# ramanathanlab/distllm

Measured on NVIDIA H100. Metric: embedded chunks/sec @512-tok, higher is better.
Workload: dtype bf16

## Files before the change

distllm_b200/csrc/b2e_api.cu:

```cuda
#include "../../include/b2e.h"
#include "../../include/b2e_debug.h"

#include <cuda.h>
#include <cuda_runtime.h>

#include <cstdarg>
#include <cstdio>
#include <cstdlib>
#include <cstring>
#include <string>
#include <utility>
#include <vector>

#include "attention.cuh"
#include "binsearch.cuh"
#include "common.cuh"
#include "gemm.cuh"
#include "mistral_ops.cuh"
#include "pack.cuh"
#include "rowops.cuh"
#include "topk.cuh"
#include "topk_tc.cuh"

using namespace b2e;
// ... 63 lines not shown
  return B2E_OK;
}

int make_tmap_codes(CUtensorMap* tm, const void* base, uint64_t rows, uint64_t cols) {
  EncodeTiledFn fn = get_encode_fn();
  if (!fn) return fail(B2E_ERR_CUDA, "cuTensorMapEncodeTiled entry point unavailable");
  cuuint64_t dims[2] = {cols, rows};
  cuuint64_t strides[1] = {cols};
  cuuint32_t box[2] = {GEMM_BK / 2, GEMM_BN};
  cuuint32_t estr[2] = {1, 1};
  CUresult r = fn(tm, CU_TENSOR_MAP_DATA_TYPE_UINT8, 2, const_cast<void*>(base), dims, strides, box, estr,
                  CU_TENSOR_MAP_INTERLEAVE_NONE, CU_TENSOR_MAP_SWIZZLE_NONE, CU_TENSOR_MAP_L2_PROMOTION_L2_256B,
                  CU_TENSOR_MAP_FLOAT_OOB_FILL_NONE);
  if (r != CUDA_SUCCESS)
    return fail(B2E_ERR_CUDA, "cuTensorMapEncodeTiled codes(rows=%llu, cols=%llu) -> %d", (unsigned long long)rows,
                (unsigned long long)cols, (int)r);
  return B2E_OK;
}

int make_tmap_f32(CUtensorMap* tm, const void* base, uint64_t rows, uint64_t cols, uint32_t box_rows) {
  EncodeTiledFn fn = get_encode_fn();
  if (!fn) return fail(B2E_ERR_CUDA, "cuTensorMapEncodeTiled entry point unavailable");
  cuuint64_t dims[2] = {cols, rows};
  cuuint64_t strides[1] = {cols * 4};
  cuuint32_t box[2] = {32, box_rows};
  cuuint32_t estr[2] = {1, 1};
  CUresult r = fn(tm, CU_TENSOR_MAP_DATA_TYPE_FLOAT32, 2, const_cast<void*>(base), dims, strides, box, estr,
                  CU_TENSOR_MAP_INTERLEAVE_NONE, CU_TENSOR_MAP_SWIZZLE_128B, CU_TENSOR_MAP_L2_PROMOTION_L2_256B,
                  CU_TENSOR_MAP_FLOAT_OOB_FILL_NONE);
  if (r != CUDA_SUCCESS)
    return fail(B2E_ERR_CUDA, "cuTensorMapEncodeTiled f32(rows=%llu, cols=%llu, box_rows=%u) -> %d",
                (unsigned long long)rows, (unsigned long long)cols, box_rows, (int)r);
  return B2E_OK;
}

struct DeviceInfo {
  int sms = 0;
  int cc_major = 0;
  bool ok = false;
};

int device_info(int device, DeviceInfo* info) {
  int n = 0;
  if (cudaGetDeviceCount(&n) != cudaSuccess || n == 0) {
    cudaGetLastError();
    return fail(B2E_ERR_NO_DEVICE, "no CUDA device visible; libb2e has no CPU fallback");
  }
  if (device < 0 || device >= n) return fail(B2E_ERR_INVALID, "device %d out of range", device);
  cudaDeviceProp p;
  CUDA_TRY(cudaGetDeviceProperties(&p, device));
  if (p.major != 9 || p.minor != 0)
    return fail(B2E_ERR_NO_DEVICE, "device %d is sm_%d%d; libb2e is built for sm_90a only", device,
                p.major, p.minor);
  info->sms = p.multiProcessorCount;
  info->cc_major = p.major;
  info->ok = true;
  return B2E_OK;
}

int current_device_info(DeviceInfo* info) {
  int dev = 0;
  if (cudaGetDevice(&dev) != cudaSuccess) {
    cudaGetLastError();
    return fail(B2E_ERR_NO_DEVICE, "no CUDA device visible; libb2e has no CPU fallback");
  }
  static DeviceInfo cache[64];
  if (dev < 64 && cache[dev].ok) {
    *info = cache[dev];
    return B2E_OK;
  }
  int rc = device_info(dev, info);
  if (rc == B2E_OK && dev < 64) cache[dev] = *info;
  return rc;
}

template <typename Kern>
int ensure_smem_attr(Kern kern, int bytes) {
  static std::vector<std::pair<const void*, int>> done;
  int dev = 0;
  CUDA_TRY(cudaGetDevice(&dev));
  const void* key = reinterpret_cast<const void*>(kern);
  for (const auto& d : done)
    if (d.first == key && d.second == dev) return B2E_OK;
  CUDA_TRY(cudaFuncSetAttribute(kern, cudaFuncAttributeMaxDynamicSharedMemorySize, bytes));
  done.emplace_back(key, dev);
  return B2E_OK;
}

int check_gemm_shape(int M, int N, int K) {
  if (M <= 0 || N <= 0 || K <= 0) return fail(B2E_ERR_INVALID, "gemm: empty shape %dx%dx%d", M, N, K);
  if (N % 128 != 0) return fail(B2E_ERR_INVALID, "gemm: N=%d must be a multiple of 128", N);
  if (K % 64 != 0) return fail(B2E_ERR_INVALID, "gemm: K=%d must be a multiple of 64", K);
  return B2E_OK;
}

bool g_gemm_profiling = false;

int g_gemm_bn = -1;
inline int gemm_bn_override() {
  if (g_gemm_bn < 0) {
    const char* e = getenv("B2E_GEMM_BN");
    const int v = e ? atoi(e) : 0;
    g_gemm_bn = (v == 128 || v == 192) ? v : 0;
  }
  return g_gemm_bn;
}

int gemm_bn(int N, int epi, bool nf4) {
  const bool wide_ok = !nf4 && epi != B2E_EPI_SWIGLU && epi != B2E_EPI_GEGLU && N % 192 == 0;
  if (!wide_ok) return 128;
  const int forced = gemm_bn_override();
  return forced ? forced : 192;
}

struct GemmW {
  CUtensorMap tm;
  const float* absmax = nullptr;
  int bn = GEMM_BN;
};

int make_gemm_w(GemmW* w, const void* base, const float* absmax, uint64_t rows, uint64_t cols, int epi) {
  w->absmax = absmax;
  w->bn = gemm_bn((int)rows, epi, absmax != nullptr);
  return absmax ? make_tmap_codes(&w->tm, base, rows, cols / 2) : make_tmap_h16(&w->tm, base, rows, cols, w->bn);
}

template <int EPI>
int launch_gemm_epi(const CUtensorMap& ta, const GemmW& wb, void* out, const float* bias,
                    const h16* resid, int M, int N, int K, cudaStream_t st, const int* m_dev) {
  auto kern = gemm_h16_wgmma_kernel<EPI>;
  int smem = GEMM_SMEM_BYTES;
  if (N % wb.bn != 0) return fail(B2E_ERR_INVALID, "gemm: N=%d is not a multiple of its W map's tile width %d", N, wb.bn);
  if (wb.absmax) {
    kern = gemm_h16_wgmma_kernel<EPI, false, true>;
    smem = GemmPlan<true>::SMEM_BYTES;
  } else if (wb.bn == 192) {
    if constexpr (epi_is_glu(EPI)) {
      return fail(B2E_ERR_INVALID, "gemm: the gated epilogues run 128-wide tiles only");
    } else {
      kern = gemm_h16_wgmma_kernel<EPI, false, false, 192>;
      smem = GemmPlan<false, 192>::SMEM_BYTES;
      if constexpr (EPI == EPI_BIAS)
        if (g_gemm_profiling) kern = gemm_h16_wgmma_kernel<EPI, true, false, 192>;
    }
  } else if constexpr (EPI == EPI_BIAS) {
    if (g_gemm_profiling) kern = gemm_h16_wgmma_kernel<EPI, true>;
  }
  int rc = ensure_smem_attr(kern, smem);
  if (rc) return rc;
  DeviceInfo dev;
  if ((rc = current_device_info(&dev))) return rc;
  const long long tiles = (long long)(N / wb.bn) * ((M + GEMM_BM - 1) / GEMM_BM);
  if (tiles > 0x7fffffffLL) return fail(B2E_ERR_INVALID, "gemm: %lld output tiles exceed one grid", tiles);
  CUtensorMap tm_out;
  if ((rc = make_tmap_h16(&tm_out, out, M, epi_is_glu(EPI) ? N / 2 : N, GEMM_BM))) return rc;
  const unsigned grid = (unsigned)(tiles < dev.sms ? tiles : dev.sms);
  kern<<<grid, GEMM_THREADS, smem, st>>>(ta, wb.tm, tm_out, static_cast<h16*>(out), bias, resid, M, N, K, m_dev,
                                         wb.absmax);
  CUDA_TRY(cudaGetLastError());
  return B2E_OK;
}

int launch_gemm(const CUtensorMap& ta, const GemmW& tb, void* out, const float* bias,
                const void* resid, int M, int N, int K, int epi, cudaStream_t st, const int* m_dev = nullptr) {
  const h16* r = static_cast<const h16*>(resid);
  switch (epi) {
    case B2E_EPI_BIAS: return launch_gemm_epi<EPI_BIAS>(ta, tb, out, bias, r, M, N, K, st, m_dev);
    case B2E_EPI_BIAS_GELU: return launch_gemm_epi<EPI_BIAS_GELU>(ta, tb, out, bias, r, M, N, K, st, m_dev);
    case B2E_EPI_BIAS_RESID: return launch_gemm_epi<EPI_BIAS_RESID>(ta, tb, out, bias, r, M, N, K, st, m_dev);
    case B2E_EPI_SWIGLU: return launch_gemm_epi<EPI_SWIGLU>(ta, tb, out, bias, r, M, N, K, st, m_dev);
    case B2E_EPI_GEGLU: return launch_gemm_epi<EPI_GEGLU>(ta, tb, out, bias, r, M, N, K, st, m_dev);
  }
  return fail(B2E_ERR_INVALID, "unknown epilogue %d", epi);
}

template <typename T>
struct DevBuf {
  T* p = nullptr;
  size_t cap = 0;
  operator T*() const { return p; }
  int grow(size_t n, uint64_t& gen, bool zero = false) {
    if (n <= cap) return B2E_OK;
    ++gen;
    release();
    CUDA_TRY(cudaMalloc(&p, n * sizeof(T)));
    if (zero) CUDA_TRY(cudaMemset(p, 0, n * sizeof(T)));
    cap = n;
    return B2E_OK;
  }
  void release() {
    cudaFree(p);
    p = nullptr;
    cap = 0;
  }
};

struct DeviceScratch {
  int device = -1;
  uint64_t gen = 0;
};

template <typename Scratch>
int follow_device(Scratch& s) {
  int dev = 0;
  CUDA_TRY(cudaGetDevice(&dev));
  if (dev != s.device) {
    s.release();
    s.device = dev;
    ++s.gen;
  }
  return B2E_OK;
}

struct AttnScratch : DeviceScratch {
  DevBuf<float> bias;
  DevBuf<int> kv_chunks;
  DevBuf<int> plain_chunks;
  int ensure(int B, int S_pad) {
    int rc;
    if ((rc = follow_device(*this)) || (rc = bias.grow((size_t)B * S_pad, gen)) || (rc = kv_chunks.grow(B, gen)) ||
        (rc = plain_chunks.grow(B, gen)))
      return rc;
    return B2E_OK;
  }
  void release() {
    bias.release();
    kv_chunks.release();
    plain_chunks.release();
  }
};

inline int attn_s_pad(int S) { return (S + AT_KC - 1) / AT_KC * AT_KC; }

int attention_prepare(AttnScratch& sc, const int64_t* mask, int B, int S, cudaStream_t st) {
  int rc;
  const int S_pad = attn_s_pad(S);
  if ((rc = sc.ensure(B, S_pad))) return rc;
  attn_prep_kernel<<<(B + 7) / 8, 256, 0, st>>>(mask, sc.bias, sc.kv_chunks, sc.plain_chunks, B, S, S_pad);
  CUDA_TRY(cudaGetLastError());
  return B2E_OK;
}

struct SeqLayout {
  const int* cu = nullptr;
  const int* len = nullptr;
  const int* t_real = nullptr;
  const int* tok_src = nullptr;
};

struct PackBuffers : DeviceScratch {
  DevBuf<int> len_raw, ok, len;
  DevBuf<int> cu;
  DevBuf<int> t_real;
  DevBuf<int> src;
  int ensure(int B, size_t tokens) {
    int rc;
    if ((rc = follow_device(*this)) || (rc = len_raw.grow(B, gen)) || (rc = ok.grow(B, gen)) ||
        (rc = len.grow(B, gen)) || (rc = cu.grow((size_t)B + 1, gen)) || (rc = t_real.grow(2, gen)) ||
        (rc = src.grow(tokens, gen)))
      return rc;
    return B2E_OK;
  }
  void release() {
    len_raw.release(); ok.release(); len.release(); cu.release(); t_real.release(); src.release();
  }
};

template <int D, int MODE, int V>
int launch_attention_kernel(const CUtensorMap& tm, const AttnScratch& sc, void* ctx, int B, int S, int heads,
                            int kv_heads, int window, cudaStream_t st, const SeqLayout& lay) {
  using Cfg = AtCfg<D, V>;
  auto kern = attention_kernel<D, MODE, V>;
  int rc = ensure_smem_attr(kern, Cfg::SMEM_BYTES);
  if (rc) return rc;
  CUtensorMap tm_ctx = {};
  if ((V & 128) && (rc = make_tmap_h16(&tm_ctx, ctx, (uint64_t)B * S, (uint64_t)heads * D, 64, Cfg::COLS))) return rc;
  const float scale_log2e = 1.4426950408889634f / sqrtf(static_cast<float>(D));
  const long long ctas = (long long)heads * B * ((S + Cfg::QT - 1) / Cfg::QT);
  if (ctas > 0x7fffffffLL)
    return fail(B2E_ERR_INVALID, "attention: %lld CTAs (heads=%d B=%d S=%d) exceed one grid", ctas, heads, B, S);
  kern<<<(unsigned)ctas, Cfg::THREADS, Cfg::SMEM_BYTES, st>>>(tm, tm_ctx, sc.bias, sc.kv_chunks, sc.plain_chunks, B, S,
                                                    attn_s_pad(S), heads, kv_heads, window, scale_log2e, lay.cu,
                                                    lay.len, static_cast<h16*>(ctx));
  CUDA_TRY(cudaGetLastError());
  return B2E_OK;
}

constexpr int AT_DEFAULT_VARIANT = 193;
int g_att3_variant = -1;
inline int att3_variant() {
  if (g_att3_variant < 0) {
    const char* e = getenv("B2E_ATT3");
    g_att3_variant = e ? atoi(e) : AT_DEFAULT_VARIANT;
  }
  return g_att3_variant;
}

int launch_attention(const CUtensorMap& tkv, const AttnScratch& sc, void* ctx, int B, int S, int heads,
                     cudaStream_t st, int window = 0, const SeqLayout& lay = SeqLayout()) {
  const int v = att3_variant();
#define B2E_ATT(MODE, V) launch_attention_kernel<64, MODE, V>(tkv, sc, ctx, B, S, heads, heads, window, st, lay)
  if (window > 0) {
    switch (v & 192) {
      case 0: return B2E_ATT(1, 0);
      case 64: return B2E_ATT(1, 64);
      case 128: return B2E_ATT(1, 128);
      case 192: return B2E_ATT(1, 192);
    }
    return fail(B2E_ERR_INVALID, "windowed attention: variant %d has no instantiation (bits 6-7 of the variant pick "
                "0, 64, 128 or 192)", v);
  }
// ... 127 lines not shown
  NORM_ADD_RMS,
};

using TrunkFn = int (*)(B2EEncoder* e, const int64_t* ids, const int64_t* mask, const int64_t* types, int B, int S,
                        cudaStream_t st, const SeqLayout& lay);

struct Family {
  int lead, stride;
  int wqkv, wo, w1, w2;
  bool w1_gated;
  int w1_epi;
  FinalNorm norm;
  int norm_g, norm_b;
  TrunkFn trunk;
};
const Family* family(int arch);
}

struct B2EEncoder {
  B2EModelDesc desc;
  const Family* fam = nullptr;
  int full_layers = 0;
  std::vector<const void*> w;
  int device = 0;
  int sms = 0;
  DevBuf<h16> hidden, qkv, ctx, tmp, ffn;
  DevBuf<float> xres, tok_scale;
  PoolScratch pool;
  AttnScratch attn;
  PackBuffers pack;
  std::vector<GemmW> tm_wqkv, tm_wo, tm_w1, tm_w2;
  DevBuf<int64_t> stage_in;
  DevBuf<float> stage_out;
  cudaStream_t own_stream = nullptr;
  float *rope_cos = nullptr, *rope_sin = nullptr;
  float *rope_cos2 = nullptr, *rope_sin2 = nullptr;

  const void* slot(int l, int k) const { return w[fam->lead + fam->stride * l + k]; }
  const float* final_norm(int k) const {
    const int s = k ? fam->norm_b : fam->norm_g;
    if (s < 0) return nullptr;
    return (const float*)(fam->norm == NORM_POST_LN ? slot(desc.num_layers - 1, s) : w[s]);
  }
  struct StepGraph {
    int B, S, pool_kind, l2, has_types, slot;
    cudaGraphExec_t exec;
  };
  std::vector<StepGraph> graphs;
  uint64_t ws_gen = 0;
  uint64_t graphs_stamp = 0;
  uint64_t buffer_stamp() const { return ws_gen + pool.gen + attn.gen + pack.gen; }
  void drop_graphs() {
    for (auto& g : graphs) cudaGraphExecDestroy(g.exec);
    graphs.clear();
  }

  int qkv_cols() const {
    return is_decoder(desc.arch) ? (desc.heads + 2 * desc.kv_heads) * desc.head_dim : 3 * desc.hidden;
  }
  int ctx_cols() const { return is_decoder(desc.arch) ? desc.heads * desc.head_dim : desc.hidden; }
  bool has_xres() const { return desc.arch != B2E_ARCH_BERT; }
};

namespace {

size_t tokens_bytes(const B2EModelDesc& d, size_t tokens) {
  if (is_decoder(d.arch))
    return tokens * (size_t)(2 * d.hidden + (2 * d.heads + 2 * d.kv_heads) * d.head_dim + d.intermediate) * 2;
  return tokens * (size_t)(6 * d.hidden + d.intermediate) * 2;
}

int ensure_workspace(B2EEncoder* e, int B, int S) {
  const size_t tokens = (size_t)B * S, H = e->desc.hidden, I = e->desc.intermediate;
  uint64_t& gen = e->ws_gen;
  int rc;
  if ((rc = e->hidden.grow(tokens * H, gen, true)) || (rc = e->tmp.grow(tokens * H, gen, true)) ||
      (rc = e->qkv.grow(tokens * e->qkv_cols(), gen, true)) || (rc = e->ctx.grow(tokens * e->ctx_cols(), gen, true)) ||
      (rc = e->ffn.grow(tokens * I, gen, true)))
    return rc;
  if (e->has_xres() && (rc = e->xres.grow(tokens * H, gen, true))) return rc;
  if (e->desc.arch == B2E_ARCH_ESM2 && (rc = e->tok_scale.grow(B, gen))) return rc;
  if ((rc = e->pack.ensure(B, tokens))) return rc;
  return e->pool.ensure(B, S, (size_t)B * pool_nsplit(S) * e->desc.hidden);
}

int g_packing = -1;
inline bool packing_enabled() {
  if (g_packing < 0) {
    const char* e = getenv("B2E_PACKED");
    g_packing = (e && e[0] == '0') ? 0 : 1;
  }
  return g_packing == 1;
}

int pack_prepare(PackBuffers& pk, const int64_t* mask, int B, int S, bool enable, cudaStream_t st, SeqLayout* lay) {
  pack_lengths_kernel<<<(B + 7) / 8, 256, 0, st>>>(mask, pk.len_raw, pk.ok, B, S);
  pack_scan_kernel<<<1, 256, 0, st>>>(pk.len_raw, pk.ok, pk.len, pk.cu, pk.t_real, B, S, enable ? 1 : 0);
  pack_fill_kernel<<<dim3((S + 255) / 256, B), 256, 0, st>>>(pk.len, pk.cu, pk.src, B, S);
  CUDA_TRY(cudaGetLastError());
  lay->cu = pk.cu;
  lay->len = pk.len;
  lay->t_real = pk.t_real;
  lay->tok_src = pk.src;
  return B2E_OK;
}

int validate_batch(const B2EEncoder* e, int B, int S) {
  if (!e) return fail(B2E_ERR_INVALID, "null encoder handle");
  if (B <= 0 || S <= 0) return fail(B2E_ERR_INVALID, "empty batch B=%d S=%d", B, S);
  int cur = -1;
  if (cudaGetDevice(&cur) == cudaSuccess && cur != e->device)
    return fail(B2E_ERR_INVALID, "encoder lives on device %d but device %d is current", e->device, cur);
  if (S > e->desc.max_pos)
    return fail(B2E_ERR_INVALID, "S=%d exceeds max_position_embeddings=%d", S, e->desc.max_pos);
  return B2E_OK;
}

struct TrunkMaps {
  CUtensorMap hidden, ctx, ffn, qkv;
};

int trunk_prologue(B2EEncoder* e, const int64_t* mask, int B, int S, cudaStream_t st, TrunkMaps* tm) {
  const B2EModelDesc& d = e->desc;
  const int M = B * S;
  int rc;
  if ((rc = attention_prepare(e->attn, mask, B, S, st))) return rc;
  if ((rc = make_tmap_h16(&tm->hidden, e->hidden, M, d.hidden, 128))) return rc;
  if ((rc = make_tmap_h16(&tm->ctx, e->ctx, M, e->ctx_cols(), 128))) return rc;
  if ((rc = make_tmap_h16(&tm->ffn, e->ffn, M, d.intermediate, 128))) return rc;
  if (is_decoder(d.arch)) return B2E_OK;
  return make_tmap_h16(&tm->qkv, e->qkv, M, e->qkv_cols(), AT_KC, d.head_dim);
}

int run_bert_trunk(B2EEncoder* e, const int64_t* ids, const int64_t* mask, const int64_t* types,
                   int B, int S, cudaStream_t st, const SeqLayout& lay) {
  const B2EModelDesc& d = e->desc;
  const int M = B * S, H = d.hidden, I = d.intermediate;
  int rc;
  DISPATCH_H(H, (embed_layernorm_kernel<HW><<<row_blocks(M), ROW_THREADS, 0, st>>>(
                     ids, types, (const float*)e->w[0], (const float*)e->w[1], (const float*)e->w[2],
                     (const float*)e->w[3], (const float*)e->w[4], e->hidden, M, S, d.eps, lay.t_real,
                     lay.tok_src)));
  CUDA_TRY(cudaGetLastError());

  TrunkMaps tm;
  if ((rc = trunk_prologue(e, mask, B, S, st, &tm))) return rc;

  for (int l = 0; l < d.num_layers; ++l) {
    if ((rc = launch_gemm(tm.hidden, e->tm_wqkv[l], e->qkv, (const float*)e->slot(l, 1), nullptr, M,
                          3 * H, H, B2E_EPI_BIAS, st, lay.t_real)))
      return rc;
    if ((rc = launch_attention_bidir(tm.qkv, e->attn, e->ctx, B, S, d.heads, d.head_dim, st, lay)))
      return rc;
    if ((rc = launch_gemm(tm.ctx, e->tm_wo[l], e->tmp, (const float*)e->slot(l, 3), nullptr, M, H, H,
                          B2E_EPI_BIAS, st, lay.t_real)))
      return rc;
    DISPATCH_H(H, (layernorm_kernel<HW, h16><<<row_blocks(M), ROW_THREADS, 0, st>>>(
                       e->tmp, e->hidden, (const float*)e->slot(l, 4), (const float*)e->slot(l, 5),
                       e->hidden, M, d.eps, lay.t_real)));
    if ((rc = launch_gemm(tm.hidden, e->tm_w1[l], e->ffn, (const float*)e->slot(l, 7), nullptr, M, I,
                          H, B2E_EPI_BIAS_GELU, st, lay.t_real)))
      return rc;
    if ((rc = launch_gemm(tm.ffn, e->tm_w2[l], e->tmp, (const float*)e->slot(l, 9), nullptr, M, H, I,
                          B2E_EPI_BIAS, st, lay.t_real)))
      return rc;
    if (l + 1 < d.num_layers) {
      DISPATCH_H(H, (layernorm_kernel<HW, h16><<<row_blocks(M), ROW_THREADS, 0, st>>>(
                         e->tmp, e->hidden, (const float*)e->slot(l, 10), (const float*)e->slot(l, 11),
                         e->hidden, M, d.eps, lay.t_real)));
    }
  }
  CUDA_TRY(cudaGetLastError());
  return B2E_OK;
}

int run_esm_trunk(B2EEncoder* e, const int64_t* ids, const int64_t* mask, const int64_t*, int B, int S,
                  cudaStream_t st, const SeqLayout& lay) {
  const B2EModelDesc& d = e->desc;
  const int M = B * S, H = d.hidden, I = d.intermediate, L = d.num_layers;
  const int mask_token = d.reserved - 1;
  int rc;
  esm_token_scale_kernel<<<(B + 7) / 8, 256, 0, st>>>(ids, mask, e->tok_scale, B, S, mask_token);
  DISPATCH_H(H, (esm_embed_kernel<HW><<<row_blocks(M), ROW_THREADS, 0, st>>>(
                     ids, mask, (const float*)e->w[0], e->tok_scale, e->xres, M, S, mask_token, lay.t_real,
                     lay.tok_src)));
  CUDA_TRY(cudaGetLastError());
  TrunkMaps tm;
  if ((rc = trunk_prologue(e, mask, B, S, st, &tm))) return rc;

  DISPATCH_H(H, (add_layernorm_kernel<HW, h16><<<row_blocks(M), ROW_THREADS, 0, st>>>(
                     e->xres, nullptr, (const float*)e->slot(0, 0), (const float*)e->slot(0, 1), e->hidden,
                     M, d.eps, lay.t_real)));
  const long long rope_work = (long long)M * d.heads * 2;
  for (int l = 0; l < L; ++l) {
    if ((rc = launch_gemm(tm.hidden, e->tm_wqkv[l], e->qkv, (const float*)e->slot(l, 3), nullptr, M,
                          3 * H, H, B2E_EPI_BIAS, st, lay.t_real)))
      return rc;
    if (d.head_dim == 32) {
      rope_halves_kernel<16><<<(unsigned)((rope_work * 2 + 255) / 256), 256, 0, st>>>(
          e->qkv, e->rope_cos, e->rope_sin, M, S, 2 * d.heads, 3 * H, lay.t_real, lay.tok_src);
    } else {
      rope_halves_kernel<32><<<(unsigned)((rope_work * 4 + 255) / 256), 256, 0, st>>>(
          e->qkv, e->rope_cos, e->rope_sin, M, S, 2 * d.heads, 3 * H, lay.t_real, lay.tok_src);
    }
    if ((rc = launch_attention_bidir(tm.qkv, e->attn, e->ctx, B, S, d.heads, d.head_dim, st, lay)))
      return rc;
    if ((rc = launch_gemm(tm.ctx, e->tm_wo[l], e->tmp, (const float*)e->slot(l, 5), nullptr, M, H, H,
                          B2E_EPI_BIAS, st, lay.t_real)))
      return rc;
    DISPATCH_H(H, (add_layernorm_kernel<HW, h16><<<row_blocks(M), ROW_THREADS, 0, st>>>(
                       e->xres, e->tmp, (const float*)e->slot(l, 6), (const float*)e->slot(l, 7), e->hidden,
                       M, d.eps, lay.t_real)));
    if ((rc = launch_gemm(tm.hidden, e->tm_w1[l], e->ffn, (const float*)e->slot(l, 9), nullptr, M, I, H,
                          B2E_EPI_BIAS_GELU, st, lay.t_real)))
      return rc;
    if ((rc = launch_gemm(tm.ffn, e->tm_w2[l], e->tmp, (const float*)e->slot(l, 11), nullptr, M, H, I,
                          B2E_EPI_BIAS, st, lay.t_real)))
      return rc;
    if (l + 1 < L) {
      DISPATCH_H(H, (add_layernorm_kernel<HW, h16><<<row_blocks(M), ROW_THREADS, 0, st>>>(
                         e->xres, e->tmp, (const float*)e->slot(l + 1, 0), (const float*)e->slot(l + 1, 1),
                         e->hidden, M, d.eps, lay.t_real)));
    }
  }
  CUDA_TRY(cudaGetLastError());
  return B2E_OK;
}

int run_mistral_trunk(B2EEncoder* e, const int64_t* ids, const int64_t* mask, const int64_t*, int B, int S,
                      cudaStream_t st, const SeqLayout& lay) {
  const B2EModelDesc& d = e->desc;
  const int M = B * S, H = d.hidden, I = d.intermediate, L = d.num_layers;
  const int QC = e->qkv_cols(), CC = e->ctx_cols();
  int rc;
  DISPATCH_H(H, (mistral_embed_kernel<HW><<<row_blocks(M), ROW_THREADS, 0, st>>>(
                     ids, (const float*)e->w[0], e->xres, M, lay.t_real, lay.tok_src)));
  CUDA_TRY(cudaGetLastError());
  TrunkMaps tm;
  if ((rc = trunk_prologue(e, mask, B, S, st, &tm))) return rc;

  DISPATCH_H(H, (add_rmsnorm_kernel<HW, h16><<<row_blocks(M), ROW_THREADS, 0, st>>>(
                     e->xres, nullptr, (const float*)e->slot(0, 0), e->hidden, M, d.eps, lay.t_real)));
  const int n_rot = d.heads + d.kv_heads;
  const long long rope_work = (long long)M * n_rot;
  for (int l = 0; l < L; ++l) {
    if ((rc = launch_gemm(tm.hidden, e->tm_wqkv[l], e->qkv, nullptr, nullptr, M, QC, H, B2E_EPI_BIAS, st, lay.t_real)))
      return rc;
    if (d.arch == B2E_ARCH_QWEN3) {
      qk_rmsnorm_rope_kernel<<<(unsigned)((rope_work * 8 + 255) / 256), 256, 0, st>>>(
          e->qkv, (const float*)e->slot(l, 6), (const float*)e->slot(l, 7), e->rope_cos, e->rope_sin, M, S, d.heads,
          d.kv_heads, QC, d.eps, lay.t_real, lay.tok_src);
    } else {
      rope_halves_kernel<64><<<(unsigned)((rope_work * 8 + 255) / 256), 256, 0, st>>>(
          e->qkv, e->rope_cos, e->rope_sin, M, S, n_rot, QC, lay.t_real, lay.tok_src);
    }
    if ((rc = launch_attention_causal_d128(e->qkv, e->attn, e->ctx, B, S, d.heads, d.kv_heads,
                                           d.sliding_window, st, lay)))
      return rc;
    if ((rc = launch_gemm(tm.ctx, e->tm_wo[l], e->tmp, nullptr, nullptr, M, H, CC, B2E_EPI_BIAS, st, lay.t_real)))
      return rc;
    DISPATCH_H(H, (add_rmsnorm_kernel<HW, h16><<<row_blocks(M), ROW_THREADS, 0, st>>>(
                       e->xres, e->tmp, (const float*)e->slot(l, 3), e->hidden, M, d.eps, lay.t_real)));
    if ((rc = launch_gemm(tm.hidden, e->tm_w1[l], e->ffn, nullptr, nullptr, M, 2 * I, H,
                          B2E_EPI_SWIGLU, st, lay.t_real)))
      return rc;
    if ((rc = launch_gemm(tm.ffn, e->tm_w2[l], e->tmp, nullptr, nullptr, M, H, I, B2E_EPI_BIAS, st, lay.t_real)))
      return rc;
    if (l + 1 < L) {
      DISPATCH_H(H, (add_rmsnorm_kernel<HW, h16><<<row_blocks(M), ROW_THREADS, 0, st>>>(
                         e->xres, e->tmp, (const float*)e->slot(l + 1, 0), e->hidden, M, d.eps, lay.t_real)));
    }
  }
  CUDA_TRY(cudaGetLastError());
  return B2E_OK;
}

int run_modernbert_trunk(B2EEncoder* e, const int64_t* ids, const int64_t* mask, const int64_t*, int B, int S,
                         cudaStream_t st, const SeqLayout& lay) {
  const B2EModelDesc& d = e->desc;
  const int M = B * S, H = d.hidden, I = d.intermediate, L = d.num_layers;
  int rc;
  DISPATCH_H(H, (modernbert_embed_kernel<HW><<<row_blocks(M), ROW_THREADS, 0, st>>>(
                     ids, (const float*)e->w[0], (const float*)e->w[1], (const float*)e->w[2], e->xres,
                     e->hidden, M, d.eps, lay.t_real, lay.tok_src)));
  CUDA_TRY(cudaGetLastError());
  TrunkMaps tm;
  if ((rc = trunk_prologue(e, mask, B, S, st, &tm))) return rc;
  const long long rope_work = (long long)M * d.heads * 2;
  for (int l = 0; l < L; ++l) {
    const bool global = (l % d.global_every) == 0;
    if (l > 0) {
      DISPATCH_H(H, (add_layernorm_kernel<HW, h16><<<row_blocks(M), ROW_THREADS, 0, st>>>(
                         e->xres, e->tmp, (const float*)e->slot(l, 0), (const float*)e->slot(l, 1), e->hidden, M,
                         d.eps, lay.t_real)));
    }
    if ((rc = launch_gemm(tm.hidden, e->tm_wqkv[l], e->qkv, nullptr, nullptr, M, 3 * H, H, B2E_EPI_BIAS, st, lay.t_real)))
      return rc;
    rope_halves_kernel<32><<<(unsigned)((rope_work * 4 + 255) / 256), 256, 0, st>>>(
        e->qkv, global ? e->rope_cos : e->rope_cos2, global ? e->rope_sin : e->rope_sin2, M, S, 2 * d.heads,
        3 * H, lay.t_real, lay.tok_src);
    if ((rc = launch_attention(tm.qkv, e->attn, e->ctx, B, S, d.heads, st,
                               global ? 0 : d.sliding_window, lay)))
      return rc;
    if ((rc = launch_gemm(tm.ctx, e->tm_wo[l], e->tmp, nullptr, nullptr, M, H, H, B2E_EPI_BIAS, st, lay.t_real)))
      return rc;
    DISPATCH_H(H, (add_layernorm_kernel<HW, h16><<<row_blocks(M), ROW_THREADS, 0, st>>>(
                       e->xres, e->tmp, (const float*)e->slot(l, 4), (const float*)e->slot(l, 5), e->hidden, M,
                       d.eps, lay.t_real)));
    if ((rc = launch_gemm(tm.hidden, e->tm_w1[l], e->ffn, nullptr, nullptr, M, 2 * I, H, B2E_EPI_GEGLU, st, lay.t_real)))
      return rc;
    if ((rc = launch_gemm(tm.ffn, e->tm_w2[l], e->tmp, nullptr, nullptr, M, H, I, B2E_EPI_BIAS, st, lay.t_real)))
      return rc;
  }
  CUDA_TRY(cudaGetLastError());
  return B2E_OK;
}

constexpr Family kFamilies[] = {
    {5, 12, 0, 2, 6, 8, false, B2E_EPI_BIAS_GELU, NORM_POST_LN, 10, 11, run_bert_trunk},
    {3, 12, 2, 4, 8, 10, false, B2E_EPI_BIAS_GELU, NORM_ADD_LN, 1, 2, run_esm_trunk},
    {2, 6, 1, 2, 4, 5, true, B2E_EPI_SWIGLU, NORM_ADD_RMS, 1, -1, run_mistral_trunk},
// ... 943 lines not shown
```

distllm_b200/csrc/gemm.cuh:

```cuda
#pragma once

#include "common.cuh"

namespace b2e {

enum GemmEpi : int { EPI_BIAS = 0, EPI_BIAS_GELU = 1, EPI_BIAS_RESID = 2, EPI_SWIGLU = 3, EPI_GEGLU = 4 };
__host__ __device__ constexpr bool epi_is_glu(int epi) { return epi == EPI_SWIGLU || epi == EPI_GEGLU; }

constexpr int GEMM_BM = 128;
constexpr int GEMM_BN = 128;
constexpr int GEMM_BK = 64;
constexpr int GEMM_STAGES = 5;
constexpr int GEMM_THREADS = 384;
constexpr int GEMM_PRODUCER_REGS = 40, GEMM_CONSUMER_REGS = 232;
constexpr int GEMM_A_BYTES = GEMM_BM * GEMM_BK * 2;
constexpr int GEMM_STAGE_BYTES = GEMM_A_BYTES + GEMM_BN * GEMM_BK * 2;
constexpr int GEMM_OUT_BOX = GEMM_BM * 64 * 2;
constexpr int GEMM_OUT_OFFSET = GEMM_STAGES * GEMM_STAGE_BYTES;
constexpr int GEMM_BAR_OFFSET = GEMM_OUT_OFFSET + 2 * 2 * GEMM_OUT_BOX;
constexpr int GEMM_SMEM_BYTES = GEMM_BAR_OFFSET + 16 * GEMM_STAGES + 1024;
static_assert(GEMM_SMEM_BYTES <= 232448, "shared memory of one SM");
constexpr int GEMM_BAR_TURN = 1, GEMM_BAR_STAGE = 3, GEMM_BAR_NF4 = 5;

constexpr int GEMM_NF4_RAW = 4;
constexpr int GEMM_NF4_CODE_BYTES = GEMM_BN * GEMM_BK / 2;
constexpr int GEMM_NF4_RAW_BYTES = GEMM_NF4_CODE_BYTES + GEMM_BN * 4;

template <bool NF4, int BN = GEMM_BN>
struct GemmPlan {
  static_assert(BN == 128 || BN == 192, "tile widths");
  static_assert(!NF4 || BN == 128, "the NF4 producer writes one W row per thread of its warpgroup");
  static constexpr int STAGE_BYTES = GEMM_A_BYTES + BN * GEMM_BK * 2;
  static constexpr int OUT_BOXES = BN / 64;
  static constexpr int STAGES = NF4 ? 4 : BN == 192 ? 3 : GEMM_STAGES;
  static constexpr int OUT_OFFSET = STAGES * STAGE_BYTES;
  static constexpr int RAW_OFFSET = OUT_OFFSET + 2 * OUT_BOXES * GEMM_OUT_BOX;
  static constexpr int BAR_OFFSET = RAW_OFFSET + (NF4 ? GEMM_NF4_RAW * GEMM_NF4_RAW_BYTES : 0);
  static constexpr int TABLE_OFFSET = BAR_OFFSET + 16 * STAGES + (NF4 ? 8 * GEMM_NF4_RAW : 0);
  static constexpr int SMEM_BYTES = TABLE_OFFSET + (NF4 ? 16 * 4 : 0) + 1024;
  static constexpr int PRODUCER_REGS = NF4 ? 56 : BN == 192 ? 24 : GEMM_PRODUCER_REGS;
  static constexpr int CONSUMER_REGS = NF4 ? 224 : BN == 192 ? 240 : GEMM_CONSUMER_REGS;
  static_assert(128 * PRODUCER_REGS + 256 * CONSUMER_REGS <= GEMM_THREADS * 168, "registers the CTA holds");
  static_assert(SMEM_BYTES <= 232448, "shared memory of one SM");
};
static_assert(GemmPlan<false>::SMEM_BYTES == GEMM_SMEM_BYTES && GemmPlan<false>::BAR_OFFSET == GEMM_BAR_OFFSET &&
              GemmPlan<false>::STAGE_BYTES == GEMM_STAGE_BYTES, "the 16-bit plan");

__constant__ uint32_t kNf4CodeBits[16] = {
    0xbf800000u, 0xbf3239b1u, 0xbf066b30u, 0xbeca32a0u, 0xbe91a24du, 0xbe3d353fu, 0xbdba7871u, 0x00000000u,
    0x3da2faffu, 0x3e24cae3u, 0x3e7c04ddu, 0x3ead033au, 0x3ee1a4b8u, 0x3f1007abu, 0x3f3913b3u, 0x3f800000u,
};

__device__ __forceinline__ float gelu_erf_fast(float x) {
  const float xc = fminf(fmaxf(x, -5.65685f), 5.65685f);
  const float v = xc * xc;
  float q = fmaf(v, -1.35688221e-05f, -1.95764464e-04f);
  q = fmaf(v, q, 3.65498251e-02f);
  q = fmaf(v, q, 7.97818838e-01f);
  float t;
  asm("tanh.approx.f32 %0, %1;" : "=f"(t) : "f"(xc * q));
  const float h = 0.5f * x;
  return fmaf(h, t, h);
}

__device__ __forceinline__ float gelu_erf(float x) {
  const float ax = fabsf(x);
  float t;
  asm("rcp.approx.ftz.f32 %0, %1;" : "=f"(t) : "f"(fmaf(0.3275911f * 0.70710678f, ax, 1.0f)));
  float p = fmaf(t, 1.061405429f, -1.453152027f);
  p = fmaf(t, p, 1.421413741f);
  p = fmaf(t, p, -0.284496736f);
  p = fmaf(t, p, 0.254829592f);
  p *= t;
  const float e = fast_exp2(ax * ax * (-0.5f * 1.4426950408889634f));
  return fmaxf(x, 0.0f) - 0.5f * ax * p * e;
}

__device__ __forceinline__ float silu(float x) {
  float r;
  asm("rcp.approx.ftz.f32 %0, %1;" : "=f"(r) : "f"(1.0f + fast_exp2(-1.4426950408889634f * x)));
  return x * r;
}


__device__ long long* g_gemm_clock = nullptr;

struct GemmTiles {
  int first, stride, count, n_tiles;
};
template <int BN>
__device__ __forceinline__ GemmTiles gemm_tiles(int M, int N) {
  const int n_tiles = N / BN;
  const int tiles = n_tiles * ((M + GEMM_BM - 1) / GEMM_BM);
  const int first = static_cast<int>(blockIdx.x), stride = static_cast<int>(gridDim.x);
  return {first, stride, first < tiles ? (tiles - 1 - first) / stride + 1 : 0, n_tiles};
}

__device__ __forceinline__ float ld_shared_const_f32(uint32_t addr) {
  float v;
  asm("ld.shared.f32 %0, [%1];" : "=f"(v) : "r"(addr));
  return v;
}
__device__ __forceinline__ float ld_shared_f32(uint32_t addr) {
  float v;
  asm volatile("ld.shared.f32 %0, [%1];" : "=f"(v) : "r"(addr) : "memory");
  return v;
}
__device__ __forceinline__ uint4 ld_shared_v4(uint32_t addr) {
  uint4 v;
  asm volatile("ld.shared.v4.u32 {%0, %1, %2, %3}, [%4];" : "=r"(v.x), "=r"(v.y), "=r"(v.z), "=r"(v.w) : "r"(addr)
               : "memory");
  return v;
}
__device__ __forceinline__ void st_shared_v4(uint32_t addr, uint32_t a, uint32_t b, uint32_t c, uint32_t d) {
  asm volatile("st.shared.v4.b32 [%0], {%1, %2, %3, %4};" ::"r"(addr), "r"(a), "r"(b), "r"(c), "r"(d) : "memory");
}

__device__ __forceinline__ void gemm_nf4_producer(const CUtensorMap* tm_a, const CUtensorMap* tm_codes,
                                                  const float* __restrict__ absmax, const GemmTiles& tl, int N,
                                                  int kblocks, uint32_t sb, uint32_t full_bar, uint32_t empty_bar) {
  using P = GemmPlan<true>;
  const int p = static_cast<int>(threadIdx.x) - 256;
  const uint32_t raw0 = sb + P::RAW_OFFSET;
  const uint32_t raw_bar = empty_bar + 8u * P::STAGES;
  const uint32_t table = sb + P::TABLE_OFFSET;
  const int total = tl.count * kblocks;
  int ld = 0, ld_tile = 0, ld_kb = 0;
  auto load_raw = [&]() {
    const int slot = ld % GEMM_NF4_RAW;
    const int tile = tl.first + ld_tile * tl.stride;
    const int n0 = (tile % tl.n_tiles) * GEMM_BN;
    const uint32_t dst = raw0 + slot * GEMM_NF4_RAW_BYTES, bar = raw_bar + 8u * slot;
    mbar_expect_tx(bar, GEMM_NF4_RAW_BYTES);
    tma_load_2d(dst, tm_codes, bar, ld_kb * (GEMM_BK / 2), n0);
    bulk_load_1d(dst + GEMM_NF4_CODE_BYTES, absmax + static_cast<size_t>(ld_kb) * N + n0, GEMM_BN * 4, bar);
    ++ld;
    if (++ld_kb == kblocks) { ld_kb = 0; ++ld_tile; }
  };
  if (p == 0) {
    tma_prefetch_desc(tm_a);
    tma_prefetch_desc(tm_codes);
    while (ld < total && ld < GEMM_NF4_RAW) load_raw();
  }
  int stage = 0, slot = 0;
  uint32_t phase = 0, raw_phase = 0;
  for (int i = 0; i < tl.count; ++i) {
    const int m0 = ((tl.first + i * tl.stride) / tl.n_tiles) * GEMM_BM;
    for (int kb = 0; kb < kblocks; ++kb) {
      mbar_wait(empty_bar + 8u * stage, phase ^ 1u);
      const uint32_t dst = sb + stage * GEMM_STAGE_BYTES;
      const uint32_t fb = full_bar + 8u * stage;
      if (p == 0) {
        mbar_expect_tx(fb, GEMM_A_BYTES);
        tma_load_2d(dst, tm_a, fb, kb * GEMM_BK, m0);
      }
      mbar_wait(raw_bar + 8u * slot, raw_phase);
      const uint32_t src = raw0 + slot * GEMM_NF4_RAW_BYTES;
      const uint4 c0 = ld_shared_v4(src + 32 * p), c1 = ld_shared_v4(src + 32 * p + 16);
      const float s = ld_shared_f32(src + GEMM_NF4_CODE_BYTES + 4 * p);
      const uint32_t words[8] = {c0.x, c0.y, c0.z, c0.w, c1.x, c1.y, c1.z, c1.w};
      const uint32_t row = dst + GEMM_A_BYTES + 128 * p;
#pragma unroll
      for (int c = 0; c < 8; ++c) {
        uint32_t v[4];
#pragma unroll
        for (int b = 0; b < 4; ++b) {
          const uint32_t byte = (words[c] >> (8 * b)) & 0xffu;
          const float lo = __fmul_rn(ld_shared_const_f32(table + ((byte >> 4) << 2)), s);
          const float hi = __fmul_rn(ld_shared_const_f32(table + ((byte & 15u) << 2)), s);
          v[b] = pack_h16x2(lo, hi);
        }
        st_shared_v4(row + ((c ^ (p & 7)) << 4), v[0], v[1], v[2], v[3]);
      }
      fence_proxy_async_smem();
      named_bar_sync(GEMM_BAR_NF4, 128);
      if (p == 0) {
        mbar_arrive(fb);
        if (ld < total) load_raw();
      }
      if (++stage == P::STAGES) { stage = 0; phase ^= 1u; }
      if (++slot == GEMM_NF4_RAW) { slot = 0; raw_phase ^= 1u; }
    }
  }
}

template <int EPI, bool TL = false, bool NF4 = false, int BN = GEMM_BN>
__global__ void __launch_bounds__(GEMM_THREADS, 1)
gemm_h16_wgmma_kernel(const __grid_constant__ CUtensorMap tm_a,
                      const __grid_constant__ CUtensorMap tm_b,
                      const __grid_constant__ CUtensorMap tm_out,
                      h16* __restrict__ out, const float* __restrict__ bias, const h16* __restrict__ resid,
                      int M, int N, int K, const int* __restrict__ m_dev, const float* __restrict__ absmax) {
  using P = GemmPlan<NF4, BN>;
  static_assert(!epi_is_glu(EPI) || BN == 128, "the gated epilogues pair gate and up within a 128-row W tile");
  if (m_dev != nullptr) M = __ldg(m_dev);
  const GemmTiles tl = gemm_tiles<BN>(M, N);
  extern __shared__ uint8_t smem_raw[];
  const uint32_t sb = (smem_u32(smem_raw) + 1023u) & ~1023u;
  const uint32_t full_bar = sb + P::BAR_OFFSET;
  const uint32_t empty_bar = full_bar + 8u * P::STAGES;
  const int warp = threadIdx.x >> 5;
  const int kblocks = K / GEMM_BK;

  if (threadIdx.x == 0) {
    for (int s = 0; s < P::STAGES; ++s) {
      mbar_init(full_bar + 8u * s, NF4 ? 2 : 1);
      mbar_init(empty_bar + 8u * s, 1);
    }
    if constexpr (NF4)
      for (int s = 0; s < GEMM_NF4_RAW; ++s) mbar_init(empty_bar + 8u * (P::STAGES + s), 1);
    mbar_fence_init();
  }
  if constexpr (NF4)
    if (threadIdx.x < 16) st_shared_u32(sb + P::TABLE_OFFSET + 4 * threadIdx.x, kNf4CodeBits[threadIdx.x]);
  __syncthreads();

  long long* clk = (TL && blockIdx.x == 0) ? g_gemm_clock : nullptr;
  if (warp >= 8) {
    asm volatile("setmaxnreg.dec.sync.aligned.u32 %0;" ::"n"(P::PRODUCER_REGS));
    if constexpr (NF4) {
      gemm_nf4_producer(&tm_a, &tm_b, absmax, tl, N, kblocks, sb, full_bar, empty_bar);
    } else if (warp == 8 && elect_one()) {
      tma_prefetch_desc(&tm_a);
      tma_prefetch_desc(&tm_b);
      int stage = 0, n = 0;
      uint32_t phase = 0;
      for (int i = 0; i < tl.count; ++i) {
        const int tile = tl.first + i * tl.stride;
        const int m0 = (tile / tl.n_tiles) * GEMM_BM, n0 = (tile % tl.n_tiles) * BN;
        for (int kb = 0; kb < kblocks; ++kb, ++n) {
          mbar_wait(empty_bar + 8u * stage, phase ^ 1u);
          const uint32_t dst = sb + stage * P::STAGE_BYTES;
          const uint32_t fb = full_bar + 8u * stage;
          mbar_expect_tx(fb, P::STAGE_BYTES);
          tma_load_2d(dst, &tm_a, fb, kb * GEMM_BK, m0);
          tma_load_2d(dst + GEMM_A_BYTES, &tm_b, fb, kb * GEMM_BK, n0);
          if (TL && clk != nullptr && n < 256) clk[n] = clock64();
          if (++stage == P::STAGES) { stage = 0; phase ^= 1u; }
        }
      }
    }
    return;
  }

  asm volatile("setmaxnreg.inc.sync.aligned.u32 %0;" ::"n"(P::CONSUMER_REGS));
  const int wg = warp >> 2;
  const int t = threadIdx.x & 127;
  const int quad = t & 3;
  const int r_lo = 16 * (t >> 5) + ((t & 31) >> 2);
  const uint32_t stg = sb + P::OUT_OFFSET + wg * (P::OUT_BOXES * GEMM_OUT_BOX);
  int retired = 0;
  for (int i = wg; i < tl.count; i += 2) {
    const int tile = tl.first + i * tl.stride;
    const int m0 = (tile / tl.n_tiles) * GEMM_BM, n_blk = tile % tl.n_tiles;
    float acc[2][BN / 2];
#pragma unroll
    for (int x = 0; x < BN / 2; ++x) acc[0][x] = acc[1][x] = 0.0f;
    if (i > 0) named_bar_sync(GEMM_BAR_TURN + wg, 256);
    const int it = i * kblocks;
    int stage = it % P::STAGES;
    uint32_t phase = (it / P::STAGES) & 1u;
    int prev = -1;
    for (int kb = 0; kb < kblocks; ++kb) {
      mbar_wait(full_bar + 8u * stage, phase);
      const uint32_t a_addr = sb + stage * P::STAGE_BYTES;
      const uint64_t a0 = make_smem_desc_sw128(a_addr), a1 = make_smem_desc_sw128(a_addr + 64 * 128);
      const uint64_t b_desc = make_smem_desc_sw128(a_addr + GEMM_A_BYTES);
      reg_fence(acc[0]);
      reg_fence(acc[1]);
      wgmma_fence();
#pragma unroll
      for (int k = 0; k < GEMM_BK / 16; ++k) {
        if constexpr (BN == 192) {
          wgmma_64x192_ss(acc[0], a0 + 2u * k, b_desc + 2u * k, (kb | k) != 0);
          wgmma_64x192_ss(acc[1], a1 + 2u * k, b_desc + 2u * k, (kb | k) != 0);
        } else {
          wgmma_64x128_ss(acc[0], a0 + 2u * k, b_desc + 2u * k, (kb | k) != 0);
          wgmma_64x128_ss(acc[1], a1 + 2u * k, b_desc + 2u * k, (kb | k) != 0);
        }
      }
      wgmma_commit();
      reg_fence(acc[0]);
      reg_fence(acc[1]);
      wgmma_wait<1>();
      reg_fence(acc[0]);
      reg_fence(acc[1]);
      if (prev >= 0 && t == 0) mbar_arrive(empty_bar + 8u * prev);
      if (TL && clk != nullptr && wg == 0 && t == 0 && retired < 256) clk[256 + retired] = clock64();
      ++retired;
      prev = stage;
      if (++stage == P::STAGES) { stage = 0; phase ^= 1u; }
    }
    if (i + 1 < tl.count) named_bar_arrive(GEMM_BAR_TURN + (wg ^ 1), 256);
    wgmma_wait<0>();
    reg_fence(acc[0]);
    reg_fence(acc[1]);
    if (t == 0) mbar_arrive(empty_bar + 8u * prev);

    const bool staged = m0 + GEMM_BM <= M;
    if (staged) {
      if (t == 0) tma_store_wait_read<0>();
      named_bar_sync(GEMM_BAR_STAGE + wg, 128);
    }
    if constexpr (epi_is_glu(EPI)) {
      const int n_out = N / 2;
#pragma unroll
      for (int j = 0; j < 8; ++j)
#pragma unroll
        for (int h = 0; h < 2; ++h)
#pragma unroll
          for (int half = 0; half < 2; ++half) {
            const int r = 64 * h + r_lo + 8 * half;
            const float g0 = acc[h][4 * j + 2 * half], g1 = acc[h][4 * j + 2 * half + 1];
            const float u0 = acc[h][4 * (j + 8) + 2 * half], u1 = acc[h][4 * (j + 8) + 2 * half + 1];
            float v0, v1;
            if (EPI == EPI_GEGLU) {
              v0 = gelu_erf_fast(g0) * u0;
              v1 = gelu_erf_fast(g1) * u1;
            } else {
              v0 = silu(g0) * u0;
              v1 = silu(g1) * u1;
            }
            if (staged)
              st_shared_u32(stg + r * 128 + ((j ^ (r & 7)) << 4) + 4 * quad, pack_h16x2(v0, v1));
            else if (m0 + r < M)
              *reinterpret_cast<uint32_t*>(out + static_cast<size_t>(m0 + r) * n_out + n_blk * (GEMM_BN / 2) +
                                           8 * j + 2 * quad) = pack_h16x2(v0, v1);
          }
    } else {
      const int col0 = n_blk * BN + 2 * quad;
#pragma unroll
      for (int j = 0; j < BN / 8; ++j) {
        const float2 b = bias != nullptr ? __ldg(reinterpret_cast<const float2*>(bias + col0 + 8 * j))
                                         : make_float2(0.0f, 0.0f);
#pragma unroll
        for (int h = 0; h < 2; ++h)
#pragma unroll
          for (int half = 0; half < 2; ++half) {
            const int r = 64 * h + r_lo + 8 * half;
            if (!staged && m0 + r >= M) continue;
            float v0 = acc[h][4 * j + 2 * half], v1 = acc[h][4 * j + 2 * half + 1];
            if (bias != nullptr) {
              v0 += b.x;
              v1 += b.y;
            }
            if (EPI == EPI_BIAS_GELU) {
              v0 = gelu_erf_fast(v0);
              v1 = gelu_erf_fast(v1);
            }
            const size_t off = static_cast<size_t>(m0 + r) * N + col0 + 8 * j;
            if (EPI == EPI_BIAS_RESID) {
              const float2 rv = unpack_h16x2(*reinterpret_cast<const uint32_t*>(resid + off));
              v0 += rv.x;
              v1 += rv.y;
            }
            if (staged)
              st_shared_u32(stg + (j >> 3) * GEMM_OUT_BOX + r * 128 + (((j & 7) ^ (r & 7)) << 4) + 4 * quad,
                            pack_h16x2(v0, v1));
            else
              *reinterpret_cast<uint32_t*>(out + off) = pack_h16x2(v0, v1);
          }
      }
    }
    if (staged) {
      fence_proxy_async_smem();
      named_bar_sync(GEMM_BAR_STAGE + wg, 128);
      if (t == 0) {
        if constexpr (epi_is_glu(EPI)) {
          tma_store_2d(&tm_out, stg, n_blk * (GEMM_BN / 2), m0);
        } else {
#pragma unroll
          for (int b = 0; b < P::OUT_BOXES; ++b) tma_store_2d(&tm_out, stg + b * GEMM_OUT_BOX, n_blk * BN + 64 * b, m0);
        }
        tma_store_commit();
      }
    }
  }
  if (t == 0) tma_store_wait_all();
}

}
```

Measured before the change: 4466.

## Fuse residual add into O-proj and FFN-down GEMM epilogues via TMA-loaded residual tiles

The BERT trunk's attention-output and FFN-down GEMMs now use the bias+residual epilogue, so the following layernorm no longer reads the residual separately. The residual tile is prefetched by TMA into the output staging buffer at the start of each tile, guarded by a new mbarrier, and read from shared memory in the epilogue instead of from global memory. This removes one activation read from each layernorm and hides the residual load behind the mainloop. In exchange it adds barrier bookkeeping and reuses the staging buffer, which must first wait for prior TMA stores to finish reading it. The non-staged path still reads the residual from shared memory, which may not be valid for partial tiles.

```diff
diff --git a/distllm_b200/csrc/b2e_api.cu b/distllm_b200/csrc/b2e_api.cu
--- a/distllm_b200/csrc/b2e_api.cu
+++ b/distllm_b200/csrc/b2e_api.cu
@@ -239,11 +239,16 @@
   if ((rc = current_device_info(&dev))) return rc;
   const long long tiles = (long long)(N / wb.bn) * ((M + GEMM_BM - 1) / GEMM_BM);
   if (tiles > 0x7fffffffLL) return fail(B2E_ERR_INVALID, "gemm: %lld output tiles exceed one grid", tiles);
-  CUtensorMap tm_out;
+  CUtensorMap tm_out, tm_resid;
   if ((rc = make_tmap_h16(&tm_out, out, M, epi_is_glu(EPI) ? N / 2 : N, GEMM_BM))) return rc;
+  if (EPI == EPI_BIAS_RESID) {
+    if ((rc = make_tmap_h16(&tm_resid, resid, M, N, GEMM_BM))) return rc;
+  } else {
+    tm_resid = tm_out;
+  }
   const unsigned grid = (unsigned)(tiles < dev.sms ? tiles : dev.sms);
-  kern<<<grid, GEMM_THREADS, smem, st>>>(ta, wb.tm, tm_out, static_cast<h16*>(out), bias, resid, M, N, K, m_dev,
-                                         wb.absmax);
+  kern<<<grid, GEMM_THREADS, smem, st>>>(ta, wb.tm, tm_out, static_cast<h16*>(out), bias, M, N, K, m_dev, wb.absmax,
+                                         tm_resid);
   CUDA_TRY(cudaGetLastError());
   return B2E_OK;
 }
@@ -677,21 +682,22 @@
       return rc;
     if ((rc = launch_attention_bidir(tm.qkv, e->attn, e->ctx, B, S, d.heads, d.head_dim, st, lay)))
       return rc;
-    if ((rc = launch_gemm(tm.ctx, e->tm_wo[l], e->tmp, (const float*)e->slot(l, 3), nullptr, M, H, H,
-                          B2E_EPI_BIAS, st, lay.t_real)))
+    if ((rc = launch_gemm(tm.ctx, e->tm_wo[l], e->tmp, (const float*)e->slot(l, 3), e->hidden, M, H, H,
+                          B2E_EPI_BIAS_RESID, st, lay.t_real)))
       return rc;
     DISPATCH_H(H, (layernorm_kernel<HW, h16><<<row_blocks(M), ROW_THREADS, 0, st>>>(
-                       e->tmp, e->hidden, (const float*)e->slot(l, 4), (const float*)e->slot(l, 5),
+                       e->tmp, nullptr, (const float*)e->slot(l, 4), (const float*)e->slot(l, 5),
                        e->hidden, M, d.eps, lay.t_real)));
     if ((rc = launch_gemm(tm.hidden, e->tm_w1[l], e->ffn, (const float*)e->slot(l, 7), nullptr, M, I,
                           H, B2E_EPI_BIAS_GELU, st, lay.t_real)))
       return rc;
-    if ((rc = launch_gemm(tm.ffn, e->tm_w2[l], e->tmp, (const float*)e->slot(l, 9), nullptr, M, H, I,
-                          B2E_EPI_BIAS, st, lay.t_real)))
-      return rc;
-    if (l + 1 < d.num_layers) {
+    const bool last = l + 1 == d.num_layers;
+    if ((rc = launch_gemm(tm.ffn, e->tm_w2[l], e->tmp, (const float*)e->slot(l, 9), last ? nullptr : e->hidden.p, M,
+                          H, I, last ? B2E_EPI_BIAS : B2E_EPI_BIAS_RESID, st, lay.t_real)))
+      return rc;
+    if (!last) {
       DISPATCH_H(H, (layernorm_kernel<HW, h16><<<row_blocks(M), ROW_THREADS, 0, st>>>(
-                         e->tmp, e->hidden, (const float*)e->slot(l, 10), (const float*)e->slot(l, 11),
+                         e->tmp, nullptr, (const float*)e->slot(l, 10), (const float*)e->slot(l, 11),
                          e->hidden, M, d.eps, lay.t_real)));
     }
   }
diff --git a/distllm_b200/csrc/gemm.cuh b/distllm_b200/csrc/gemm.cuh
--- a/distllm_b200/csrc/gemm.cuh
+++ b/distllm_b200/csrc/gemm.cuh
@@ -18,7 +18,7 @@
 constexpr int GEMM_OUT_BOX = GEMM_BM * 64 * 2;
 constexpr int GEMM_OUT_OFFSET = GEMM_STAGES * GEMM_STAGE_BYTES;
 constexpr int GEMM_BAR_OFFSET = GEMM_OUT_OFFSET + 2 * 2 * GEMM_OUT_BOX;
-constexpr int GEMM_SMEM_BYTES = GEMM_BAR_OFFSET + 16 * GEMM_STAGES + 1024;
+constexpr int GEMM_SMEM_BYTES = GEMM_BAR_OFFSET + 16 * GEMM_STAGES + 16 + 1024;
 static_assert(GEMM_SMEM_BYTES <= 232448, "shared memory of one SM");
 constexpr int GEMM_BAR_TURN = 1, GEMM_BAR_STAGE = 3, GEMM_BAR_NF4 = 5;
 
@@ -37,7 +37,8 @@
   static constexpr int RAW_OFFSET = OUT_OFFSET + 2 * OUT_BOXES * GEMM_OUT_BOX;
   static constexpr int BAR_OFFSET = RAW_OFFSET + (NF4 ? GEMM_NF4_RAW * GEMM_NF4_RAW_BYTES : 0);
   static constexpr int TABLE_OFFSET = BAR_OFFSET + 16 * STAGES + (NF4 ? 8 * GEMM_NF4_RAW : 0);
-  static constexpr int SMEM_BYTES = TABLE_OFFSET + (NF4 ? 16 * 4 : 0) + 1024;
+  static constexpr int RESID_BAR_OFFSET = TABLE_OFFSET + (NF4 ? 16 * 4 : 0);
+  static constexpr int SMEM_BYTES = RESID_BAR_OFFSET + 16 + 1024;
   static constexpr int PRODUCER_REGS = NF4 ? 56 : BN == 192 ? 24 : GEMM_PRODUCER_REGS;
   static constexpr int CONSUMER_REGS = NF4 ? 224 : BN == 192 ? 240 : GEMM_CONSUMER_REGS;
   static_assert(128 * PRODUCER_REGS + 256 * CONSUMER_REGS <= GEMM_THREADS * 168, "registers the CTA holds");
@@ -114,6 +115,11 @@
 }
 __device__ __forceinline__ void st_shared_v4(uint32_t addr, uint32_t a, uint32_t b, uint32_t c, uint32_t d) {
   asm volatile("st.shared.v4.b32 [%0], {%1, %2, %3, %4};" ::"r"(addr), "r"(a), "r"(b), "r"(c), "r"(d) : "memory");
+}
+__device__ __forceinline__ uint32_t ld_shared_u32(uint32_t addr) {
+  uint32_t v;
+  asm volatile("ld.shared.u32 %0, [%1];" : "=r"(v) : "r"(addr) : "memory");
+  return v;
 }
 
 __device__ __forceinline__ void gemm_nf4_producer(const CUtensorMap* tm_a, const CUtensorMap* tm_codes,
@@ -189,8 +195,8 @@
 gemm_h16_wgmma_kernel(const __grid_constant__ CUtensorMap tm_a,
                       const __grid_constant__ CUtensorMap tm_b,
                       const __grid_constant__ CUtensorMap tm_out,
-                      h16* __restrict__ out, const float* __restrict__ bias, const h16* __restrict__ resid,
-                      int M, int N, int K, const int* __restrict__ m_dev, const float* __restrict__ absmax) {
+                      h16* __restrict__ out, const float* __restrict__ bias, int M, int N, int K, const int* __restrict__ m_dev, const float* __restrict__ absmax,
+                      const __grid_constant__ CUtensorMap tm_resid) {
   using P = GemmPlan<NF4, BN>;
   static_assert(!epi_is_glu(EPI) || BN == 128, "the gated epilogues pair gate and up within a 128-row W tile");
   if (m_dev != nullptr) M = __ldg(m_dev);
@@ -209,6 +215,10 @@
     }
     if constexpr (NF4)
       for (int s = 0; s < GEMM_NF4_RAW; ++s) mbar_init(empty_bar + 8u * (P::STAGES + s), 1);
+    if constexpr (EPI == EPI_BIAS_RESID) {
+      mbar_init(sb + P::RESID_BAR_OFFSET, 1);
+      mbar_init(sb + P::RESID_BAR_OFFSET + 8u, 1);
+    }
     mbar_fence_init();
   }
   if constexpr (NF4)
@@ -250,12 +260,23 @@
   const int r_lo = 16 * (t >> 5) + ((t & 31) >> 2);
   const uint32_t stg = sb + P::OUT_OFFSET + wg * (P::OUT_BOXES * GEMM_OUT_BOX);
   int retired = 0;
+  uint32_t resid_phase = 0;
+  const uint32_t resid_bar = sb + P::RESID_BAR_OFFSET + 8u * wg;
   for (int i = wg; i < tl.count; i += 2) {
     const int tile = tl.first + i * tl.stride;
     const int m0 = (tile / tl.n_tiles) * GEMM_BM, n_blk = tile % tl.n_tiles;
     float acc[2][BN / 2];
 #pragma unroll
     for (int x = 0; x < BN / 2; ++x) acc[0][x] = acc[1][x] = 0.0f;
+    if constexpr (EPI == EPI_BIAS_RESID) {
+      if (t == 0) {
+        tma_store_wait_read<0>();
+        mbar_expect_tx(resid_bar, P::OUT_BOXES * GEMM_OUT_BOX);
+#pragma unroll
+        for (int b = 0; b < P::OUT_BOXES; ++b)
+          tma_load_2d(stg + b * GEMM_OUT_BOX, &tm_resid, resid_bar, n_blk * BN + 64 * b, m0);
+      }
+    }
     if (i > 0) named_bar_sync(GEMM_BAR_TURN + wg, 256);
     const int it = i * kblocks;
     int stage = it % P::STAGES;
@@ -328,6 +349,10 @@
                                            8 * j + 2 * quad) = pack_h16x2(v0, v1);
           }
     } else {
+      if constexpr (EPI == EPI_BIAS_RESID) {
+        mbar_wait(resid_bar, resid_phase);
+        resid_phase ^= 1u;
+      }
       const int col0 = n_blk * BN + 2 * quad;
 #pragma unroll
       for (int j = 0; j < BN / 8; ++j) {
@@ -349,14 +374,14 @@
               v1 = gelu_erf_fast(v1);
             }
             const size_t off = static_cast<size_t>(m0 + r) * N + col0 + 8 * j;
+            const uint32_t sa = stg + (j >> 3) * GEMM_OUT_BOX + r * 128 + (((j & 7) ^ (r & 7)) << 4) + 4 * quad;
             if (EPI == EPI_BIAS_RESID) {
-              const float2 rv = unpack_h16x2(*reinterpret_cast<const uint32_t*>(resid + off));
+              const float2 rv = unpack_h16x2(ld_shared_u32(sa));
               v0 += rv.x;
               v1 += rv.y;
             }
             if (staged)
-              st_shared_u32(stg + (j >> 3) * GEMM_OUT_BOX + r * 128 + (((j & 7) ^ (r & 7)) << 4) + 4 * quad,
-                            pack_h16x2(v0, v1));
+              st_shared_u32(sa, pack_h16x2(v0, v1));
             else
               *reinterpret_cast<uint32_t*>(out + off) = pack_h16x2(v0, v1);
           }
```

After: 4468, median of 6. Within noise of the previous version (+0.1%).
